# Vanlightly/vsr-tlaplus

Hardware: AMD Instinct MI355X
Metric: distinct states/sec (whole node) + time-to-first-violation, VSR 3-replica (higher is better)
Workload: dtype u64

## Files before the change

vsr_tlaplus_amd/csrc/vsr_kernels.hpp:

```cpp
#pragma once
#include <hip/hip_runtime.h>

#include "vsr_actions.hpp"
#include "vrst_actions.hpp"
#include "vras_actions.hpp"

namespace vsr {

template <int MODEL>
struct ModelOps;
template <>
struct ModelOps<0> {
  template <bool GUARD_ONLY, typename PTR>
  static VSR_HD bool gen_(const Model& M, PTR rec, int ord, Delta& D) { return gen<GUARD_ONLY>(M, rec, ord, D); }
  template <typename PTR>
  static VSR_HD u32 guard_pre(const Model& M, PTR rec, u64 hdr, const u64* Areg, int slot, int* kind0, int info) {
    return guard_slot_pre(M, rec, hdr, Areg, slot, kind0, info);
  }
  template <typename PTR>
  static VSR_HD u32 guard(const Model& M, PTR rec, int slot, int* kind0) { return guard_slot(M, rec, slot, kind0); }
  static VSR_HD int other_kind(int) { return A_SendGetState; }
  template <typename PTR>
  static VSR_HD void hash_child_(const Model& M, PTR rec, const Delta& D, u64* Hc) { hash_child(M, rec, D, Hc); }
  template <typename PTR>
// ... 218 lines not shown
        if (cur == 0) {
          r.slot = lb + k;
          r.claimed = true;
          return r;
        }
        if (cur == fp) {
          r.slot = lb + k;
          r.reload = true;
          return r;
        }
        continue;
      }
      if (cur == fp) {
        r.slot = lb + k;
        r.meta = sk.y;
        return r;
      }
    }
    i = (lb + 4) & mask;
  }
  r.full = true;
  return r;
}

template <typename CNT>
__device__ __forceinline__ bool probe_lookup(const Slot* table, u64 mask, u64 fp, u64* meta, CNT nprobe, u64* slot_out = nullptr) {
  typedef u64 u64x2 __attribute__((ext_vector_type(2)));
  u64 i = fp & mask;
  {
    const u64x2 sk = *(const u64x2*)&table[i];
    nprobe.home();
    if (sk.x == fp) {
      *meta = sk.y;
      if (slot_out) *slot_out = i;
      return true;
    }
    if (sk.x == 0) return false;
    i = (i + 1) & mask;
  }
  for (u32 lines = 0; lines < 2048; lines++) {
    const u64 lb = i & ~(u64)3;
    const u64x2* lp = (const u64x2*)&table[lb];
    const u64x2 s0 = lp[0], s1 = lp[1], s2 = lp[2], s3 = lp[3];
#pragma unroll
    for (int k = 0; k < 4; k++) {
      if (lb + k < i) continue;
      const u64x2 sk = k == 0 ? s0 : k == 1 ? s1 : k == 2 ? s2 : s3;
      nprobe.extra();
      if (sk.x == fp) {
        *meta = sk.y;
        if (slot_out) *slot_out = lb + k;
        return true;
      }
      if (sk.x == 0) return false;
    }
    i = (lb + 4) & mask;
  }
  return false;
}

template <typename CNT>
__device__ __forceinline__ u64 table_claim(Slot* table, u64 mask, u64 fp, u64 key, int level, bool* found_old,
                                           CNT nprobe, bool* full) {
  const Probe p = probe_insert(table, mask, fp, nprobe);
  *full = p.full;
  *found_old = true;
  if (p.full) return 0;
  if (!p.claimed) {
    const u64 m = p.reload ? __hip_atomic_load(&table[p.slot].meta, __ATOMIC_RELAXED, __HIP_MEMORY_SCOPE_AGENT) : p.meta;
    if (meta_level(m) < level || m < key) return p.slot;
  }
  const u64 prev = atomicMin((unsigned long long*)&table[p.slot].meta, (unsigned long long)key);
  *found_old = prev < key;
  return p.slot;
}

template <typename CNT>
__device__ __forceinline__ void table_claim_fused(Slot* table, u64 mask, u64 fp, u64 key, int level, bool* claimed, u64* prev_meta,
                                                  CNT nprobe, bool* full) {
  const Probe p = probe_insert(table, mask, fp, nprobe);
  *full = p.full;
  *claimed = p.claimed;
  *prev_meta = META_EMPTY;
  if (p.full) return;
  if (!p.claimed) {
    const u64 m = p.reload ? __hip_atomic_load(&table[p.slot].meta, __ATOMIC_RELAXED, __HIP_MEMORY_SCOPE_AGENT) : p.meta;
    if (meta_level(m) < level) return;
    if (m != META_EMPTY && m < key) {
      *prev_meta = m;
      return;
    }
  }
  *prev_meta = atomicMin((unsigned long long*)&table[p.slot].meta, (unsigned long long)key);
}

template <int SPEC>
__device__ __forceinline__ void specialise(Model& M, const Model& Marg) {
  constexpr int MODEL = SPEC / 1000, S = SPEC % 1000;
  if constexpr (S != 0) {
    constexpr int SR = S / 100, SC = (S / 10) % 10, SN = S % 10;
    M.R = SR;
    M.C = SC;
    M.n = SN;
    if constexpr (MODEL == 0) {
      M.wpr = 1 + (SR + 2) / 2;
      M.m0 = 4 * SR + SR * SC * SN;
      if (Marg.np == 1) M.np = 1;
      else M.np = SN == 1 ? 1 : SN == 2 ? 2 : 6;
    } else {
      M.wpr = MODEL == 1 ? 1 : 2;
      M.m0 = 4 * SR + SR * SN;
      M.np = 1;
    }
    M.h0 = 1 + SR * M.wpr;
    M.fixed = M.h0 + M.np + VSR_PAD_WORDS;
    M.pitab[0] = 0x24u;
    if (SN == 2) M.pitab[1] = 0x21u;
    if (SN == 3) { M.pitab[1] = 0x18u; M.pitab[2] = 0x21u; M.pitab[3] = 0x09u; M.pitab[4] = 0x12u; M.pitab[5] = 0x06u; }
  }
}

constexpr int EXPAND_GENERAL = 0;
constexpr int EXPAND_PLAIN = 1;
constexpr int EXPAND_MODES = 2;
constexpr int EXPAND_REGEN_BITS = 3;
constexpr int EXPAND_INSERT = 4;
constexpr int EXPAND_PLAIN5 = 5;
constexpr int EXPAND_PROBE = 6;
constexpr int expand_occ(bool fused, int spec, int plain) {
  return !fused ? 3 : spec == 0 ? 2 : (plain == EXPAND_PLAIN5 || plain == EXPAND_PROBE) ? VSR_OCC + 1 : VSR_OCC;
}
template <bool FUSED, int SPEC = 0, int PLAIN = EXPAND_GENERAL>
__global__ void __launch_bounds__(VSR_BLOCK, expand_occ(FUSED, SPEC, PLAIN))
k_expand(Model Marg, const u64* __restrict__ fr_words, const u64* __restrict__ fr_off, u64 n_parents, int level, int rank,
         Slot* table, u64 tmask, u64* pending, u64 pending_cap, LevelCtl* ctl, int stride, int world_arg, u64* cand_send,
         u64 cand_cap, u32 pchunk ,
         u64* nx_words, u64 nx_words_cap, u64* nx_off, u64 nx_cap, u64* lvl_fp, u32 ichunk, u32 wchunk, int tile, u32 ccap ,
         u64* filter, u64 fmask, u64* cand_idx, u32 cchunk ,
         int mode_arg, u64 p_offset ,
         const WSet* wset, u32 wepoch) {
  constexpr bool IS_PLAIN = PLAIN == EXPAND_PLAIN || PLAIN == EXPAND_PLAIN5;
  const int mode = IS_PLAIN ? (int)MODE_NORMAL : PLAIN == EXPAND_REGEN_BITS ? (int)MODE_REGEN : PLAIN == EXPAND_INSERT ? (int)MODE_INSERT
                 : PLAIN == EXPAND_PROBE ? (int)MODE_PROBE : (mode_arg & 0xFF);
  const bool no_footprint = !IS_PLAIN && PLAIN != EXPAND_PROBE && (mode_arg & MODE_NO_FOOTPRINT) != 0;
  const int world = PLAIN != EXPAND_GENERAL ? 1 : world_arg;
  Model M = Marg;
  specialise<SPEC>(M, Marg);
  typedef ModelOps<SPEC / 1000> Ops;
  extern __shared__ u64 smem[];
  u64* s_rec = smem;
  u32* s_cand = (u32*)(smem + tile * stride);
  u32* s_cand2 = s_cand + ccap;
  __shared__ u32 s_ncand, s_napply, s_dead, s_maxbag, s_maxbag_out, s_skip, s_nsurv, s_risky, s_ntotal;
  constexpr int TILE_MAX = (FUSED && SPEC % 1000 != 0 && (SPEC % 1000) / 100 <= 3) ? 64 : VSR_TILE_MAX;
  constexpr bool COOP = FUSED && IS_PLAIN;
  constexpr bool REDO_OK = FUSED && (IS_PLAIN || PLAIN == EXPAND_PROBE);
  __shared__ u32 s_alive[TILE_MAX];
  __shared__ u64 s_ref[TILE_MAX];
  __shared__ u64 s_pfp[TILE_MAX];
  __shared__ u32 s_kcount[16], s_kbase[16];
  __shared__ int s_slotinfo[64];
  __shared__ unsigned long long s_fxs[2];
  __shared__ unsigned long long s_acc[32];
  __shared__ u64 s_chunk_base;
  __shared__ u32 s_chunk_used, s_tile_base, s_tile_cursor;
  __shared__ u64 s_ich_base, s_wch_base;
  __shared__ u32 s_ich_used, s_wch_used, s_tile_ibase, s_tile_wbase, s_tile_icur, s_tile_wcur, s_wneed;
  __shared__ unsigned long long s_cstate[8];
  constexpr bool fused = FUSED;
  constexpr u64 CS_NONE = ((u64)1 << 40) - 1;

  const int tid = threadIdx.x, lane = tid & 63;
#if VSR_WAVE_DIAG
  u64 wd_wait = 0;
  const u64 wd_t0 = __builtin_readcyclecounter();
  __shared__ unsigned long long s_wd[8];
  if (tid < 8) s_wd[tid] = 0;
#endif
  const u64 ntiles = (n_parents + tile - 1) / tile;
  const int tshift = 31 - __clz(tile);
  if (tid < 32) s_acc[tid] = 0;
  if (tid < 2) s_fxs[tid] = 0;
  if (tid == 0) s_maxbag_out = 0;
  if (tid < 64) s_slotinfo[tid] = (SPEC / 1000 == 0 && tid < M.m0) ? slot_info(M, tid) : 0;
  if (tid == 0) {
    s_chunk_base = 0; s_chunk_used = pchunk;
    s_ich_base = 0; s_ich_used = ichunk; s_wch_base = 0; s_wch_used = wchunk;
  }
  if (tid < 8) s_cstate[tid] = (CS_NONE << 24) | cchunk;
  VSR_SYNC_G(0);

  __shared__ u64 s_tile_cur;
  u64 my_next = 0;
  __shared__ u32 s_tile_left;
  const u32 tbatch = ntiles >= (u64)gridDim.x * 16 ? (u32)VSR_TILE_BATCH : 1u;
  if (tid == 0) { my_next = atomicAdd((unsigned long long*)&ctl->tile_cursor, 1ull) * (u64)tbatch; s_tile_left = tbatch - 1; }
  __shared__ u32 s_over;
  if (tid == 0) s_over = 0;
  for (;;) {
    if (tid == 0) {
      s_tile_cur = my_next;
      if (my_next < ntiles) {
        const u32 left = s_tile_left;
        if (left) { my_next++; s_tile_left = left - 1; }
        else { my_next = atomicAdd((unsigned long long*)&ctl->tile_cursor, 1ull) * (u64)tbatch; s_tile_left = tbatch - 1; }
      }
    }
    const u64 t_0 = VSR_CLK();
    if (tid == 0) { s_ncand = 0; s_dead = 0; s_maxbag = 0; s_wneed = 0; s_skip = 0; s_nsurv = 0; s_over = 0; if (!IS_PLAIN) s_risky = 0; }
    if (tid < tile) s_alive[tid] = 0;
    if (tid < 16) s_kcount[tid] = 0;
    VSR_SYNC_G(0);
    u64 tile_i = s_tile_cur;
    tile_i = ((u64)(u32)__builtin_amdgcn_readfirstlane((int)(u32)(tile_i >> 32)) << 32) | (u32)__builtin_amdgcn_readfirstlane((int)(u32)tile_i);
    if (tile_i >= ntiles) break;
    u64 p_base = tile_i * (u64)tile;
    int np_tile = (int)((n_parents - p_base) < (u64)tile ? (n_parents - p_base) : (u64)tile);
    if constexpr (REDO_OK) {
      if (mode_arg & MODE_REDO_LIST) {
        const u64 e = ((const u64*)p_offset)[tile_i >> 1];
        const int cnt = (int)(e >> 48);
        int half = 1;
        while (half * 2 < cnt) half *= 2;
        p_base = (e & (((u64)1 << 48) - 1)) + ((tile_i & 1) ? (u64)half : 0);
        np_tile = (tile_i & 1) ? cnt - half : half;
      }
      p_base = ((u64)(u32)__builtin_amdgcn_readfirstlane((int)(u32)(p_base >> 32)) << 32) | (u32)__builtin_amdgcn_readfirstlane((int)(u32)p_base);
      np_tile = __builtin_amdgcn_readfirstlane(np_tile);
    }
    u32 cbits[2] = {0u, 0u};
    if constexpr (PLAIN == EXPAND_REGEN_BITS) {
      const int pm = tid & (tile - 1), gg = tid >> tshift, GG = VSR_BLOCK >> tshift;
      if (pm < np_tile) {
        const u32* row = (const u32*)filter + (p_offset + p_base + (u64)pm) * fmask;
#pragma unroll
        for (int q = 0; q < 2; q++)
          if ((u64)(gg + q * GG) < fmask) cbits[q] = row[gg + q * GG];
      }
    }

    if (tid < np_tile) {
      const u64 ref = fr_off[p_base + tid];
      s_ref[tid] = ref;
      if (ref) atomicMax(&s_maxbag, (u32)((int)(ref & 255) - M.fixed));
      if ((int)(ref & 255) > stride) raise_error(ctl, ERR_INTERNAL, (p_base + (u64)tid) << 16);
    }
    constexpr int SG = VSR_BLOCK / 16;
    for (int half = 0; half < tile; half += 4 * SG)
      for (int wbase = 0; wbase < stride; wbase += 64) {
        u64 v[4][4];
        u64 refq[4];
#pragma unroll
        for (int q = 0; q < 4; q++) {
          const int p = half + (tid >> 4) + SG * q;
          refq[q] = p < np_tile ? fr_off[p_base + (u64)p] : 0;
        }
#pragma unroll
        for (int q = 0; q < 4; q++) {
          const u64 ref = refq[q];
          const u64 off = ref >> 8;
          const int len = (int)(ref & 255) < stride ? (int)(ref & 255) : stride;
#pragma unroll
          for (int j = 0; j < 4; j++) {
            const int k = wbase + (tid & 15) + 16 * j;
            v[q][j] = k < len ? fr_words[off + k] : 0;
          }
        }
#pragma unroll
        for (int q = 0; q < 4; q++) {
          const int p = half + (tid >> 4) + SG * q;
          const int len = (int)(refq[q] & 255) < stride ? (int)(refq[q] & 255) : stride;
#pragma unroll
          for (int j = 0; j < 4; j++) {
            const int k = wbase + (tid & 15) + 16 * j;
            if (k < len) s_rec[p * stride + k] = v[q][j];
          }
        }
      }
    VSR_SYNC_G(2);
    if (tid < np_tile && s_ref[tid] != 0) {
      const u64* r0 = s_rec + tid * stride;
      u64 pf;
      u32 pa;
      canonical_fp(M, r0[0], r0 + M.h0, &pf, &pa);
      s_pfp[tid] = pf;
    }

    const u64 t_1 = VSR_CLK();
    {
      const int nslots = M.m0 + (int)s_maxbag;
      const int nitems = nslots << tshift;
      const int p_mine = tid & (tile - 1);
      const bool mine_valid = p_mine < np_tile && s_ref[p_mine] != 0;
      const u64* rec_mine = s_rec + p_mine * stride;
      u64 Areg[6] = {0, 0, 0, 0, 0, 0};
      u64 hdr_mine = 0;
      if (mine_valid) {
        hdr_mine = rec_mine[0];
#pragma unroll
        for (int r = 1; r <= 5; r++)
          if (r <= M.R) Areg[r] = rec_mine[1 + (r - 1) * M.wpr];
      }
      const u32 PRIV = PLAIN == EXPAND_PROBE ? 0u : (ccap - (u32)VSR_BLOCK) / VSR_BLOCK;
      const u32 shared0 = PRIV * VSR_BLOCK;
      for (u32 k = tid; k < ccap; k += VSR_BLOCK) s_cand[k] = ~0u;
      VSR_SYNC_G(3);
      u32 nmine = 0;
      bool alive = false;
      if constexpr (SPEC / 1000 == 0) {
        auto emit = [&](int kind, int p, int ord) {
          atomicAdd(&s_kcount[kind], 1u);
          if constexpr (PLAIN == EXPAND_PROBE) {
            if (!((Ops::probe_actions() >> kind) & 1u)) { s_alive[p] = 1; return; }
          }
          u32 idx;
          if (nmine < PRIV) idx = (u32)tid * PRIV + nmine;
          else idx = shared0 + atomicAdd(&s_ncand, 1u);
          nmine++;
          if (idx < ccap) s_cand[idx] = ((u32)kind << 18) | ((u32)p << 11) | (u32)ord;
          else s_ncand = 0x40000000u;
          s_alive[p] = 1;
        };
        const int G = VSR_BLOCK >> tshift, g = tid >> tshift;
        if constexpr (PLAIN == EXPAND_REGEN_BITS) {
          if (mine_valid) {
#pragma unroll
            for (int q = 0; q < 2; q++) {
              u32 bits = cbits[q];
              while (bits) {
                const int b = __ffs((int)bits) - 1;
                bits &= bits - 1;
                const int ord = 32 * (g + q * G) + b;
                int kind;
                if (ord < M.m0) {
                  kind = ord < M.R ? A_TimerSendSVC : ord < 2 * M.R ? A_SendDVC : ord < 3 * M.R ? A_SendSV : ord < 4 * M.R ? A_ExecuteOp : A_ReceiveClientRequest;
                } else {
                  const int q2 = ord - M.m0, j = q2 / (M.R + 1), k2 = q2 - j * (M.R + 1);
                  int kind0 = 0;
                  (void)Ops::guard(M, rec_mine, M.m0 + j, &kind0);
                  kind = k2 == 0 ? kind0 : Ops::other_kind(kind0);
                }
                emit(kind, p_mine, ord);
              }
            }
          }
        } else {
        u64 lut[6] = {0, 0, 0, 0, 0, 0};
        if (mine_valid) {
#pragma unroll
          for (int r = 1; r <= 5; r++)
            if (r <= M.R) lut[r] = prefilter_lut(M, Areg[r], r);
          for (int r = g + 1; r <= M.R; r += G) {
            u32 m = rep_slots_mask(M, rec_mine, hdr_mine, areg_of(Areg, r), r);
            while (m) {
              const int b = __ffs((int)m) - 1;
              m &= m - 1;
              const int kind = b == 0 ? A_TimerSendSVC : b == 1 ? A_SendDVC : b == 2 ? A_SendSV : b == 3 ? A_ExecuteOp : A_ReceiveClientRequest;
              emit(kind, p_mine, b < 4 ? b * M.R + (r - 1) : 4 * M.R + (r - 1) * M.C * M.n + (b - 4));
            }
          }
        }
        u16* s_surv = (u16*)s_cand2;
        const int nmsg_mine = mine_valid ? hdr_nmsg(hdr_mine) : 0;
        const int maxbag = (int)s_maxbag;
        const int jbatch = (int)((2u * ccap) >> tshift);
        for (int j0 = 0; j0 < maxbag; j0 += jbatch) {
          const int j1 = j0 + jbatch < maxbag ? j0 + jbatch : maxbag;
          for (int jj = j0; jj < j1; jj += G) {
            const int j = jj + g;
            bool pass = false;
            if (j < j1 && j < nmsg_mine) {
              const u64 w = rec_mine[M.fixed + j];
              const int r = m_dest(w);
              const u64 l = r == 1 ? lut[1] : r == 2 ? lut[2] : r == 3 ? lut[3] : r == 4 ? lut[4] : lut[5];
              pass = m_count(w) != 0 && ((l >> (w & 63)) & 1);
              if (!IS_PLAIN && PLAIN != EXPAND_REGEN_BITS && PLAIN != EXPAND_INSERT && mode == MODE_PROBE && m_count(w) == 3) s_risky = 1;
            }
            const u64 bal = __ballot(pass);
            if (bal) {
              u32 base = 0;
              if (lane == 0) base = atomicAdd(&s_nsurv, (u32)__popcll(bal));
              base = (u32)__builtin_amdgcn_readfirstlane((int)base);
              if (pass) s_surv[base + (u32)__popcll(bal & (((u64)1 << lane) - 1))] = (u16)((p_mine << 8) | j);
            }
          }
          VSR_SYNC_G(4);
          const u32 nsurv = s_nsurv;
          for (u32 i = tid; i < nsurv; i += VSR_BLOCK) {
            const int p = s_surv[i] >> 8, j = s_surv[i] & 255;
            int kind0 = 0;
            u32 mask = Ops::guard(M, s_rec + p * stride, M.m0 + j, &kind0);
            const int ordbase = M.m0 + j * (M.R + 1);
            while (mask) {
              const int k = __ffs((int)mask) - 1;
              mask &= mask - 1;
              emit(k == 0 ? kind0 : Ops::other_kind(kind0), p, ordbase + k);
            }
          }
          if (j1 < maxbag) {
            VSR_SYNC_G(4);
            if (tid == 0) s_nsurv = 0;
            VSR_SYNC_G(4);
          }
        }
        }
      } else
      {
      for (int item0 = tid; item0 < nitems; item0 += 4 * VSR_BLOCK) {
        u32 masks[4];
        int kinds[4];
#pragma unroll
        for (int u = 0; u < 4; u++) {
          const int item = item0 + u * VSR_BLOCK;
          const int slot = item >> tshift;
          masks[u] = 0;
          kinds[u] = 0;
          if (item < nitems && mine_valid) masks[u] = Ops::guard_pre(M, rec_mine, hdr_mine, Areg, slot, &kinds[u], s_slotinfo[slot & 63]);
        }
#pragma unroll
        for (int u = 0; u < 4; u++) {
          u32 mask = masks[u];
          if (!mask) continue;
          const int slot = (item0 + u * VSR_BLOCK) >> tshift;
          const int ordbase = slot < M.m0 ? slot : M.m0 + (slot - M.m0) * (M.R + 1);
          alive = true;
          while (mask) {
            const int k = __ffs((int)mask) - 1;
            mask &= mask - 1;
            const int kind = k == 0 ? kinds[u] : Ops::other_kind(kinds[u]);
            atomicAdd(&s_kcount[kind], 1u);
            u32 idx;
            if (nmine < PRIV) idx = (u32)tid * PRIV + nmine;
            else idx = shared0 + atomicAdd(&s_ncand, 1u);
            nmine++;
            if (idx < ccap) s_cand[idx] = ((u32)kind << 18) | ((u32)p_mine << 11) | (u32)(ordbase + k);
            else s_ncand = 0x40000000u;
          }
        }
      }
      if (alive) s_alive[p_mine] = 1;
      }
    }
    VSR_SYNC_G(5);
    if (tid < np_tile && s_alive[tid] == 0 && s_ref[tid] != 0) atomicAdd(&s_dead, 1u);
    if (tid == 0) {
      if (s_ncand >= 0x40000000u) {
        bool listed = false;
        if constexpr (REDO_OK) {
          if (np_tile > 1) {
            const u64 k = atomicAdd((unsigned long long*)&ctl->n_redo, 1ull);
            if (k < ctl->redo_cap) { ((u64*)ctl->redo_out)[k] = p_base | ((u64)np_tile << 48); listed = true; s_over = 1; }
          }
        }
        if (!listed) raise_error(ctl, ERR_FRONTIER_FULL, p_base);
      }
      u32 acc = 0;
      if constexpr (!IS_PLAIN && FUSED) {
        const u32 keep = (mode == MODE_PROBE && !no_footprint) ? Ops::probe_actions() : ~0u;
        for (int a = 0; a < 16; a++)
          if ((keep >> a) & 1u) {
            s_kbase[a] = acc;
            acc += s_kcount[a];
          }
        s_napply = acc > ccap ? ccap : acc;
        if (keep != ~0u) {
          for (int a = 0; a < 16; a++)
            if (!((keep >> a) & 1u)) {
              s_kbase[a] = acc;
              acc += s_kcount[a];
            }
          if (!s_over && (s_risky || (int)s_maxbag + M.R - 1 > M.max_bag)) s_acc[15] += acc - s_napply;
        }
      } else {
        for (int a = 0; a < 16; a++) {
          s_kbase[a] = acc;
          acc += s_kcount[a];
        }
      }
      s_ncand = acc > ccap ? ccap : acc;
      if constexpr (PLAIN == EXPAND_PROBE) { s_ntotal = acc; s_ncand = s_napply; }
      if (fused) s_wneed = s_ncand * (u32)(M.fixed + (int)s_maxbag + 5);
    }
    const u64 t_2 = VSR_CLK();
    VSR_SYNC_G(6);
    const u32 ncand = s_ncand;
    if constexpr (REDO_OK) {
      if (s_over) {
        VSR_SYNC_G(6);
        continue;
      }
    }
    for (u32 c = tid; c < ccap; c += VSR_BLOCK) {
      const u32 code = s_cand[c];
      if (code == ~0u) continue;
      const u32 pos = atomicAdd(&s_kbase[code >> 18], 1u);
      if (pos < ccap) s_cand2[pos] = code;
    }
    VSR_SYNC_G(6);

    const u64 t_3 = VSR_CLK();
    if (fused && (mode == MODE_NORMAL || mode == MODE_REGEN)) {
      if (s_ich_used + ncand > ichunk) {
        const u32 used = s_ich_used;
        const u64 base = s_ich_base;
        for (u32 k = used + tid; k < ichunk; k += VSR_BLOCK) {
          nx_off[base + k] = 0;
          lvl_fp[base + k] = 0;
        }
        VSR_SYNC_G(6);
        if (tid == 0) {
          u64 nb = atomicAdd((unsigned long long*)&ctl->n_new, (unsigned long long)ichunk);
          if (nb + ichunk > nx_cap) { raise_full(ctl, nb); nb = 0; }
          s_ich_base = nb;
          s_ich_used = 0;
        }
        VSR_SYNC_G(6);
      }
      if (s_wch_used + s_wneed > wchunk) {
        VSR_SYNC_G(6);
        if (tid == 0) {
          u64 nb = atomicAdd((unsigned long long*)&ctl->words_new, (unsigned long long)wchunk);
          if (nb + wchunk > nx_words_cap) { raise_full(ctl, nb); nb = 0; }
          if (s_wneed > wchunk) { raise_error(ctl, ERR_FRONTIER_FULL, p_base); s_skip = 1; }
          s_wch_base = nb;
          s_wch_used = 0;
        }
        VSR_SYNC_G(6);
      }
      if (tid == 0) { s_tile_ibase = s_ich_used; s_tile_wbase = s_wch_used; s_tile_icur = 0; s_tile_wcur = 0; }
    } else
    if (!fused && s_chunk_used + ncand > pchunk) {
      const u32 used = s_chunk_used;
      const u64 base = s_chunk_base;
      for (u32 k = used + tid; k < pchunk && used < pchunk; k += VSR_BLOCK) pending[3 * (base + k) + 1] = ~(u64)0;
      VSR_SYNC_G(6);
      if (tid == 0) {
        u64 nb = atomicAdd((unsigned long long*)&ctl->n_pending, (unsigned long long)pchunk);
        if (nb + pchunk > pending_cap) {
          raise_error(ctl, ERR_FRONTIER_FULL, nb);
          nb = 0;
        }
        s_chunk_base = nb;
        s_chunk_used = 0;
      }
      VSR_SYNC_G(6);
    }
    const u32 ncand_apply = s_skip ? 0u : ((!IS_PLAIN && FUSED) ? s_napply : ncand);
    if (tid == 0) { s_tile_base = s_chunk_used; s_tile_cursor = 0; }
    VSR_SYNC_G(6);
    const CntLds my_probes{&s_acc[2]};
    for (u32 c = tid; c < ncand_apply; c += VSR_BLOCK) {
      const u32 code = s_cand2[c];
      const int p = (int)((code >> 11) & 127), ord = (int)(code & 2047);
      const u64* rec = s_rec + p * stride;
      Delta D;
      const u64 a_0 = VSR_CLK();
      if (!Ops::template gen_<false>(M, rec, ord, D) || D.action != (int)(code >> 18)) {
        raise_error(ctl, ERR_INTERNAL, ((p_base + (u64)p) << 16) | (u64)ord);
        continue;
      }
      if (D.err) {
        raise_error(ctl, D.err, ((p_base + (u64)p) << 16) | (u64)ord);
        continue;
      }
      if constexpr (PLAIN == EXPAND_PROBE) {
        if (Ops::invariants(M, rec, D) != 0) {
          const u64 i = atomicAdd((unsigned long long*)&ctl->n_pending, 1ull);
          if (i < pending_cap) { pending[2 * i] = origin_make(p_base + (u64)p, ord); pending[2 * i + 1] = 0; }
        }
        continue;
      }
      const u64 a_1 = VSR_CLK();
      if (!IS_PLAIN && fused && mode == MODE_PROBE && Ops::invariants(M, rec, D) == 0) continue;
      u64 Hc[6];
      Ops::hash_child_(M, rec, D, Hc);
      u64 fp;
      u32 ak;
      canonical_fp(M, D.hdr, Hc, &fp, &ak);
      const u64 key = meta_make(level, ak, s_pfp[p]);
      const u64 a_2 = VSR_CLK();
      if (tid == 0) { s_acc[10] += a_1 - a_0; s_acc[11] += a_2 - a_1; }
      if (!fused && world > 1) {
        const int owner = owner_of(fp, world);
        if (owner != rank) {
          for (int o = 0; o < world; o++)
            if (owner == o) {
              u64 i = wave_alloc(&ctl->cand_cnt[o]);
              if (i < cand_cap) {
                cand_send[2 * ((u64)o * cand_cap + i)] = fp;
                cand_send[2 * ((u64)o * cand_cap + i) + 1] = key;
                cand_idx[(u64)o * cand_cap + i] = origin_make(p_offset + p_base + (u64)p, ord);
              } else {
                raise_error(ctl, ERR_FRONTIER_FULL, i);
              }
            }
          continue;
        }
      }
      if (fused) {
        bool do_write = false, remote = false, check = false, claimed_now = false;
        u64 prev_meta = META_EMPTY;
        const int owner = world > 1 ? owner_of(fp, world) : rank;
        if (mode == MODE_PROBE) {
          u64 m = META_EMPTY;
          check = !(probe_lookup(table, tmask, fp, &m, my_probes) && meta_level(m) < level);
          if (!check) continue;
        } else if (owner != rank) {
          if (mode != MODE_REGEN) {
            u64 tag = fp ^ ((u64)(ak + 1) * 0x9E3779B97F4A7C15ull);
            if (tag == 0) tag = 1;
            u64* fs = filter + ((fp >> 6) & fmask);
            if (__hip_atomic_load(fs, __ATOMIC_RELAXED, __HIP_MEMORY_SCOPE_AGENT) == tag) continue;
            __hip_atomic_store(fs, tag, __ATOMIC_RELAXED, __HIP_MEMORY_SCOPE_AGENT);
            remote = true;
            do_write = mode == MODE_NORMAL;
          } else if (wset) {
            do_write = wset_take(wset, fp, level, wepoch);
          } else {
            remote = true;
          }
        } else if (mode == MODE_REGEN && PLAIN == EXPAND_GENERAL && wset) {
          do_write = wset_take(wset, fp, level, wepoch);
        } else if (PLAIN == EXPAND_REGEN_BITS) {
          do_write = (((const u32*)filter)[(p_offset + p_base + (u64)p) * fmask + ((u32)ord >> 5)] >> ((u32)ord & 31u)) & 1u;
        } else if (mode == MODE_REGEN) {
          u64 m = META_EMPTY;
          u64 slot_i = 0;
          do_write = probe_lookup(table, tmask, fp, &m, my_probes, &slot_i) && m == key &&
                     atomicCAS((unsigned long long*)&table[slot_i].meta, (unsigned long long)key, (unsigned long long)(key | META_TAKEN)) == key;
        } else {
          bool claimed, full;
          table_claim_fused(table, tmask, fp, key, level, &claimed, &prev_meta, my_probes, &full);
          if (full) {
            raise_error(ctl, ERR_TABLE_FULL, fp);
            continue;
          }
          do_write = claimed;
          claimed_now = claimed;
          if (PLAIN == EXPAND_GENERAL && wset && claimed && !wset_insert(wset, fp, level)) raise_error(ctl, ERR_TABLE_FULL, fp);
          if (PLAIN == EXPAND_INSERT && filter && claimed)
            atomicOr(&((u32*)filter)[(p_offset + p_base + (u64)p) * fmask + ((u32)ord >> 5)], 1u << ((u32)ord & 31u));
        }
        int bad = (check || do_write || (remote && mode == MODE_INSERT)) ? Ops::invariants(M, rec, D) : 0;
#ifdef VSRMC_TEST_HOOKS
        if constexpr (PLAIN == EXPAND_GENERAL)
          if (M.test_bad_mask && fp == M.test_bad_fp && (check || do_write || remote)) bad |= (int)M.test_bad_mask;
#endif
        if (mode == MODE_PROBE) {
          if (bad) {
// ... 16 lines not shown
            }
            atomicMin((unsigned long long*)&ctl->viol_fp, (unsigned long long)fp);
            atomicOr(&ctl->viol_mask, (u32)bad);
          }
          if ((u32)hdr_nmsg(D.hdr) > s_maxbag_out) atomicMax(&s_maxbag_out, (u32)hdr_nmsg(D.hdr));
          atomicAdd(&s_acc[9], 1ull);
          atomicXor(&s_fxs[0], (unsigned long long)fp);
          atomicAdd(&s_fxs[1], (unsigned long long)fp);
          do_write = false;
        }
        const u64 a_3 = VSR_CLK();
        if (tid == 0) s_acc[12] += a_3 - a_2;
        u64 idx = 0;
        u64 dst = 0;
        int plen = 0, clen = 0;
        if (do_write) {
          plen = (int)(s_ref[p] & 255);
          clen = M.fixed + hdr_nmsg(D.hdr);
          const u32 io = atomicAdd(&s_tile_icur, 1u);
          const u32 wo = atomicAdd(&s_tile_wcur, (u32)clen);
          idx = s_ich_base + s_tile_ibase + io;
          dst = s_wch_base + s_tile_wbase + wo;
        }
        if constexpr (COOP) {
          const u64 act = __ballot(1);
          u64 wm = __ballot(do_write);
          const int nact = __popcll(act), rnk = __popcll(act & (((u64)1 << lane) - 1));
          while (wm) {
            const int l0 = __ffsll((long long)wm) - 1;
            wm &= wm - 1;
            const int l1 = wm ? __ffsll((long long)wm) - 1 : l0;
            wm &= wm - 1;
            const int n0 = __builtin_amdgcn_readlane(plen, l0), n1 = l1 != l0 ? __builtin_amdgcn_readlane(plen, l1) : 0;
            const u64* r0 = s_rec + __builtin_amdgcn_readlane(p, l0) * stride;
            const u64* r1 = s_rec + __builtin_amdgcn_readlane(p, l1) * stride;
            u64* o0 = nx_words + readlane64(dst, l0);
            u64* o1 = nx_words + readlane64(dst, l1);
            for (int k = rnk; k < n0 || k < n1; k += nact) {
              const u64 v0 = k < n0 ? r0[k] : 0, v1 = k < n1 ? r1[k] : 0;
              if (k < n0) o0[k] = v0;
              if (k < n1) o1[k] = v1;
            }
          }
        }
        if (do_write) {
          u64* out = nx_words + dst;
          if constexpr (!COOP) {
            typedef u64 u64x2_a8 __attribute__((ext_vector_type(2), aligned(8)));
            int k = 0;
            if (plen - k >= 2) {
              u64x2_a8 cur;
              cur.x = rec[k];
              cur.y = rec[k + 1];
              for (; k + 3 < plen; k += 2) {
                u64x2_a8 nxt;
                nxt.x = rec[k + 2];
                nxt.y = rec[k + 3];
                *(u64x2_a8*)(out + k) = cur;
                cur = nxt;
              }
              *(u64x2_a8*)(out + k) = cur;
              k += 2;
            }
            for (; k + 1 < plen; k += 2) {
              u64x2_a8 v2;
              v2.x = rec[k];
              v2.y = rec[k + 1];
              *(u64x2_a8*)(out + k) = v2;
            }
            if (k < plen) out[k] = rec[k];
          }
          out[0] = D.hdr;
          u64* ob = out + 1 + (D.r - 1) * M.wpr;
          ob[0] = D.rep[0];
          if (M.wpr > 1) ob[1] = D.rep[1];
          if (M.wpr > 2) ob[2] = D.rep[2];
          if (M.wpr > 3) ob[3] = D.rep[3];
#pragma unroll
          for (int k = 0; k < 6; k++)
            if (k < M.np) out[M.h0 + k] = Hc[k];
          int a = 0;
#pragma unroll
          for (int k = 0; k < VSR_NSLOT; k++)
            if ((D.used >> k) & 1) {
              if (D.pj(k) >= 0) out[M.fixed + D.pj(k)] = D.pnew[k];
              else out[plen + (a++)] = D.pnew[k];
            }
          nx_off[idx] = (dst << 8) | (u64)clen;
          lvl_fp[idx] = fp;
          if (bad && !remote) {
            atomicMin((unsigned long long*)&ctl->viol_fp, (unsigned long long)fp);
            atomicOr(&ctl->viol_mask, (u32)bad);
          }
          if ((u32)hdr_nmsg(D.hdr) > s_maxbag_out) atomicMax(&s_maxbag_out, (u32)hdr_nmsg(D.hdr));
        }
        if (PLAIN == EXPAND_GENERAL && remote) {
          u64 i = 0;
          for (;;) {
            const unsigned long long old = atomicAdd(&s_cstate[owner], 1ull);
            const u32 pos = (u32)(old & 0xFFFFFFull);
            if (pos == cchunk) {
              u64 nb = atomicAdd((unsigned long long*)&ctl->cand_cnt[owner], (unsigned long long)cchunk);
              if (nb + cchunk > cand_cap) { raise_error(ctl, ERR_FRONTIER_FULL, nb); nb = 0; }
              const u64 ob_ = (u64)(old >> 24);
              (void)ob_;
              i = nb;
              atomicExch(&s_cstate[owner], ((unsigned long long)nb << 24) | 1ull);
              break;
            }
            if (pos < cchunk) {
              i = (u64)(old >> 24) + pos;
              break;
            }
          }
          const u64 e = (u64)owner * cand_cap + i;
          cand_send[2 * e] = fp;
          cand_send[2 * e + 1] = key;
          cand_idx[e] = mode == MODE_REGEN ? origin_make(p_base + (u64)p, ord)
                                           : cand_pack(mode == MODE_INSERT ? (u64)hdr_nmsg(D.hdr) : idx, (u32)bad);
        }
        if (prev_meta != META_EMPTY && meta_level(prev_meta) == level && meta_auxkey(prev_meta) != meta_auxkey(key)) atomicAdd(&s_acc[8], 1ull);
        if (tid == 0) s_acc[13] += VSR_CLK() - a_3;
        continue;
      }
      bool found_old, full;
      u64 slot = table_claim(table, tmask, fp, key, level, &found_old, my_probes, &full);
      if (full) {
        raise_error(ctl, ERR_TABLE_FULL, fp);
        continue;
      }
      if (!found_old) {
        const u64 active = __ballot(1);
        const int leader = __ffsll((long long)active) - 1;
        u32 b = 0;
        if (lane == leader) b = atomicAdd(&s_tile_cursor, (u32)__popcll(active));
        b = __shfl(b, leader);
        const u64 i = s_chunk_base + s_tile_base + b + (u32)__popcll(active & (((u64)1 << lane) - 1));
        pending[3 * i] = slot;
        pending[3 * i + 1] = key;
        pending[3 * i + 2] = origin_make(p_offset + p_base + (u64)p, ord);
      }
    }
    const u64 t_4 = VSR_CLK();
    VSR_SYNC_G(7);
    if (tid == 0) {
      if (fused) {
        s_ich_used += s_tile_icur;
        s_wch_used += s_tile_wcur;
        s_acc[14] += s_tile_icur;
        if (mode == MODE_NORMAL || mode == MODE_REGEN) s_acc[9] += s_tile_wcur;
      } else {
        s_chunk_used += s_tile_cursor;
      }
      s_acc[0] += PLAIN == EXPAND_PROBE ? s_ntotal : s_ncand;
      s_acc[1] += s_dead;
      if (PLAIN != EXPAND_PROBE) s_acc[2] += ncand_apply;
      const u64 t_5 = VSR_CLK();
      s_acc[3] += t_1 - t_0;
      s_acc[4] += t_2 - t_1;
      s_acc[5] += t_3 - t_2;
      s_acc[6] += t_4 - t_3;
      s_acc[7] += t_5 - t_4;
    }
    if (tid < 16) s_acc[16 + tid] += s_kcount[tid];
  }
  {
    if (fused) {
      const u32 used = s_ich_used;
      const u64 base = s_ich_base;
      for (u32 k = used + tid; k < ichunk; k += VSR_BLOCK) {
        nx_off[base + k] = 0;
        lvl_fp[base + k] = 0;
      }
      if (world > 1) {
        VSR_SYNC_G(0);
        for (int o = 0; o < world; o++) {
          const u64 st = s_cstate[o];
          const u64 base = st >> 24;
          const u32 used = (u32)(st & 0xFFFFFFull) < cchunk ? (u32)(st & 0xFFFFFFull) : cchunk;
          if (base == CS_NONE) continue;
          for (u32 k = used + tid; k < cchunk; k += VSR_BLOCK) {
            cand_send[2 * ((u64)o * cand_cap + base + k)] = 0;
            cand_send[2 * ((u64)o * cand_cap + base + k) + 1] = ~(u64)0;
          }
        }
      }
      if (tid == 0) {
        if (s_acc[8]) atomicAdd((unsigned long long*)&ctl->ties, s_acc[8]);
        if (!IS_PLAIN && s_acc[15]) atomicAdd((unsigned long long*)&ctl->limit_unchecked, s_acc[15]);
        if (s_acc[14]) atomicAdd((unsigned long long*)&ctl->n_written, s_acc[14]);
        if (s_acc[9]) atomicAdd((unsigned long long*)(mode == MODE_INSERT ? &ctl->n_new : &ctl->rec_words), s_acc[9]);
        if (s_maxbag_out) atomicMax((unsigned long long*)&ctl->max_bag, (unsigned long long)s_maxbag_out);
        if (!IS_PLAIN && (s_fxs[0] | s_fxs[1])) {
          atomicXor((unsigned long long*)&ctl->fp_xor, s_fxs[0]);
          atomicAdd((unsigned long long*)&ctl->fp_sum, s_fxs[1]);
        }
      }
    } else {
      const u32 used = s_chunk_used;
      const u64 base = s_chunk_base;
      for (u32 k = used + tid; k < pchunk; k += VSR_BLOCK) pending[3 * (base + k) + 1] = ~(u64)0;
    }
    if (tid == 0) {
      if (s_acc[0]) atomicAdd((unsigned long long*)&ctl->generated, s_acc[0]);
      if (s_acc[1]) atomicAdd((unsigned long long*)&ctl->deadlocks, s_acc[1]);
      if (s_acc[2]) atomicAdd((unsigned long long*)&ctl->probes, s_acc[2]);
    }
#if VSR_WAVE_DIAG == 3
    if (tid == 64) {
      for (int g = 0; g < 8; g++) atomicAdd((unsigned long long*)&ctl->phase_cycles[g], s_wd[g]);
      atomicAdd((unsigned long long*)&ctl->act_generated[0], (unsigned long long)(__builtin_readcyclecounter() - wd_t0));
    }
    (void)wd_wait;
#elif VSR_WAVE_DIAG
    if (lane == 0 && (tid >> 6) < 4) {
      atomicAdd((unsigned long long*)&ctl->phase_cycles[tid >> 6], (unsigned long long)wd_wait);
      atomicAdd((unsigned long long*)&ctl->phase_cycles[4 + (tid >> 6)], (unsigned long long)(__builtin_readcyclecounter() - wd_t0));
    }
#else
    if (tid >= 3 && tid < 8 && s_acc[tid]) atomicAdd((unsigned long long*)&ctl->phase_cycles[tid - 3], s_acc[tid]);
    if (tid >= 10 && tid < 13 && s_acc[tid]) atomicAdd((unsigned long long*)&ctl->phase_cycles[tid - 5], s_acc[tid]);
    if (tid == 13 && s_acc[13]) atomicAdd((unsigned long long*)&ctl->act_generated[0], s_acc[13]);
#endif
    if (tid >= 16 && tid < 32 && s_acc[tid]) atomicAdd((unsigned long long*)&ctl->act_generated[tid - 16], s_acc[tid]);
  }
}

__device__ __forceinline__ void write_child_serial(const Model& M, const u64* rec, const Delta& D, const u64* Hc, u64* dst) {
  int nmsg = hdr_nmsg(rec[0]);
  int len = M.fixed + nmsg;
  for (int k = 0; k < len; k++) dst[k] = rec[k];
  dst[0] = D.hdr;
  for (int k = 0; k < M.wpr; k++) dst[1 + (D.r - 1) * M.wpr + k] = D.rep[k];
  for (int i = 0; i < M.np; i++) dst[M.h0 + i] = Hc[i];
  int a = 0;
#pragma unroll
  for (int k = 0; k < VSR_NSLOT; k++)
    if ((D.used >> k) & 1) {
      if (D.pj(k) >= 0) dst[M.fixed + D.pj(k)] = D.pnew[k];
      else dst[M.fixed + nmsg + (a++)] = D.pnew[k];
    }
}

#define VSR_MAT_BLOCK 64
#define VSR_MAT_GROUP 16

__device__ __forceinline__ void lds_wave_sync() {
  __builtin_amdgcn_fence(__ATOMIC_RELEASE, "workgroup");
  __builtin_amdgcn_wave_barrier();
  __builtin_amdgcn_fence(__ATOMIC_ACQUIRE, "workgroup");
}

template <int SPEC>
__global__ void __launch_bounds__(VSR_MAT_BLOCK)
k_materialize(Model Marg, const u64* __restrict__ fr_words, const u64* __restrict__ fr_off, const u64* __restrict__ pending,
              u64 n_pending, Slot* table, u64* nx_words, u64 nx_words_cap, u64* nx_off, u64 nx_cap,
              u64* lvl_fp, LevelCtl* ctl, const uint8_t* __restrict__ verdict, u64* cnt_n, u64* cnt_w, int stride,
              u32 ichunk , u32 wchunk ,
              int es, const u64* __restrict__ pidx_arr) {
  Model M = Marg;
  specialise<SPEC>(M, Marg);
  typedef ModelOps<SPEC / 1000> Ops;
  extern __shared__ u64 s_slot[];
  const int lane = threadIdx.x;
  u64 idx_base = 0, w_base = 0;
  u32 idx_left = 0, w_left = 0;
  u64 cyc_fetch = 0, cyc_stage = 0, cyc_gen = 0, cyc_write = 0, rec_words = 0;
  const u64 nthreads = (u64)gridDim.x * VSR_MAT_BLOCK;
  const u64 rounds = (n_pending + nthreads - 1) / nthreads;
  for (u64 it = 0; it < rounds; it++) {
    const u64 i = it * nthreads + (u64)blockIdx.x * VSR_MAT_BLOCK + lane;
    const u64 c_0 = __builtin_readcyclecounter();
    bool win = false;
    u64 key = 0, src = 0, origin = 0;
    int plen = 0;
    if (i < n_pending) {
      key = pending[(u64)es * i + 1];
      if (key != ~(u64)0) {
        origin = pidx_arr ? pidx_arr[i] : pending[(u64)es * i + 2];
        const u64 ref = fr_off[origin_pidx(origin)];
        if (verdict) win = verdict[i] != 0;
        else win = atomicCAS((unsigned long long*)&table[pending[(u64)es * i]].meta, (unsigned long long)key,
                             (unsigned long long)(key | META_TAKEN)) == key;
        src = ref >> 8;
        plen = (int)(ref & 255);
        if (plen > stride) plen = stride;
      }
    }
    if (!win) plen = 0;
    const u64 wmask = __ballot(win);
    const u64 c_1 = __builtin_readcyclecounter();
    cyc_fetch += c_1 - c_0;
    if (wmask == 0) continue;
    for (int w = 0; w < 64; w++) {
      const int n2 = 2 * __builtin_amdgcn_readlane(plen, w);
      if (n2 == 0) continue;
      const u32* g = (const u32*)(fr_words + readlane64(src, w));
      __attribute__((address_space(3))) void* l = (__attribute__((address_space(3))) void*)(s_slot + w * stride);
      if (lane < n2) __builtin_amdgcn_global_load_lds((const __attribute__((address_space(1))) void*)(g + lane), l, 4, 0, 0);
      if (lane + 64 < n2) __builtin_amdgcn_global_load_lds((const __attribute__((address_space(1))) void*)(g + lane), l, 4, 256, 0);
      if (lane + 128 < n2) __builtin_amdgcn_global_load_lds((const __attribute__((address_space(1))) void*)(g + lane), l, 4, 512, 0);
      if (lane + 192 < n2) __builtin_amdgcn_global_load_lds((const __attribute__((address_space(1))) void*)(g + lane), l, 4, 768, 0);
    }
    asm volatile("s_waitcnt vmcnt(0)" ::: "memory");
    lds_wave_sync();
    const u64 c_2 = __builtin_readcyclecounter();
    cyc_stage += c_2 - c_1;
// ... 786 lines not shown
```

Measured before the change: 1.777 billion.

## Store private candidate slots column-major and skip full-buffer candidate clearing

```diff
diff --git a/vsr_tlaplus_amd/csrc/vsr_kernels.hpp b/vsr_tlaplus_amd/csrc/vsr_kernels.hpp
--- a/vsr_tlaplus_amd/csrc/vsr_kernels.hpp
+++ b/vsr_tlaplus_amd/csrc/vsr_kernels.hpp
@@ -394,8 +394,12 @@
   u32* s_cand = (u32*)(smem + tile * stride);
   u32* s_cand2 = s_cand + ccap;
   __shared__ u32 s_ncand, s_napply, s_dead, s_maxbag, s_maxbag_out, s_skip, s_nsurv, s_risky, s_ntotal;
+  u32& s_nlist = s_nsurv;
   constexpr int TILE_MAX = (FUSED && SPEC % 1000 != 0 && (SPEC % 1000) / 100 <= 3) ? 64 : VSR_TILE_MAX;
   constexpr bool COOP = FUSED && IS_PLAIN;
+  constexpr bool COLS = SPEC / 1000 == 0;
+  constexpr bool TWO_COLS = FUSED && SPEC != 0 && SPEC / 1000 == 0 && expand_occ(FUSED, SPEC, PLAIN) == VSR_OCC;
+  constexpr bool FLAT_STAGE = PLAIN == EXPAND_REGEN_BITS;
   constexpr bool REDO_OK = FUSED && (IS_PLAIN || PLAIN == EXPAND_PROBE);
   __shared__ u32 s_alive[TILE_MAX];
   __shared__ u64 s_ref[TILE_MAX];
@@ -497,25 +501,51 @@
           const int p = half + (tid >> 4) + SG * q;
           refq[q] = p < np_tile ? fr_off[p_base + (u64)p] : 0;
         }
-#pragma unroll
-        for (int q = 0; q < 4; q++) {
-          const u64 ref = refq[q];
-          const u64 off = ref >> 8;
-          const int len = (int)(ref & 255) < stride ? (int)(ref & 255) : stride;
+        if constexpr (FLAT_STAGE) {
+#pragma unroll
+          for (int q = 0; q < 4; q++) {
+            const u64 ref = refq[q];
+            const u64* src = fr_words + (ref >> 8);
+            const int len = (int)(ref & 255) < stride ? (int)(ref & 255) : stride;
+#pragma unroll
+            for (int j = 0; j < 4; j++) {
+              const int k = wbase + (tid & 15) + 16 * j;
+              v[q][j] = src[k < len ? k : 0];
+            }
+          }
 #pragma unroll
           for (int j = 0; j < 4; j++) {
             const int k = wbase + (tid & 15) + 16 * j;
-            v[q][j] = k < len ? fr_words[off + k] : 0;
+            if (k < stride) {
+#pragma unroll
+              for (int q = 0; q < 4; q++) {
+                const int p = half + (tid >> 4) + SG * q;
+                const int len = (int)(refq[q] & 255);
+                s_rec[p * stride + k] = k < len ? v[q][j] : 0;
+              }
+            }
           }
-        }
-#pragma unroll
-        for (int q = 0; q < 4; q++) {
-          const int p = half + (tid >> 4) + SG * q;
-          const int len = (int)(refq[q] & 255) < stride ? (int)(refq[q] & 255) : stride;
-#pragma unroll
-          for (int j = 0; j < 4; j++) {
-            const int k = wbase + (tid & 15) + 16 * j;
-            if (k < len) s_rec[p * stride + k] = v[q][j];
+        } else {
+#pragma unroll
+          for (int q = 0; q < 4; q++) {
+            const u64 ref = refq[q];
+            const u64 off = ref >> 8;
+            const int len = (int)(ref & 255) < stride ? (int)(ref & 255) : stride;
+#pragma unroll
+            for (int j = 0; j < 4; j++) {
+              const int k = wbase + (tid & 15) + 16 * j;
+              v[q][j] = k < len ? fr_words[off + k] : 0;
+            }
+          }
+#pragma unroll
+          for (int q = 0; q < 4; q++) {
+            const int p = half + (tid >> 4) + SG * q;
+            const int len = (int)(refq[q] & 255) < stride ? (int)(refq[q] & 255) : stride;
+#pragma unroll
+            for (int j = 0; j < 4; j++) {
+              const int k = wbase + (tid & 15) + 16 * j;
+              if (k < len) s_rec[p * stride + k] = v[q][j];
+            }
           }
         }
       }
@@ -529,6 +559,13 @@
     }
 
     const u64 t_1 = VSR_CLK();
+    const u32 PRIV = PLAIN == EXPAND_PROBE ? 0u : (ccap - (u32)VSR_BLOCK) / VSR_BLOCK;
+    const u32 shared0 = PRIV * VSR_BLOCK;
+    if constexpr (!COLS) {
+      for (u32 k = tid; k < ccap; k += VSR_BLOCK) s_cand[k] = ~0u;
+      VSR_SYNC_G(3);
+    }
+    u32 nmine = 0;
     {
       const int nslots = M.m0 + (int)s_maxbag;
       const int nitems = nslots << tshift;
@@ -543,11 +580,6 @@
         for (int r = 1; r <= 5; r++)
           if (r <= M.R) Areg[r] = rec_mine[1 + (r - 1) * M.wpr];
       }
-      const u32 PRIV = PLAIN == EXPAND_PROBE ? 0u : (ccap - (u32)VSR_BLOCK) / VSR_BLOCK;
-      const u32 shared0 = PRIV * VSR_BLOCK;
-      for (u32 k = tid; k < ccap; k += VSR_BLOCK) s_cand[k] = ~0u;
-      VSR_SYNC_G(3);
-      u32 nmine = 0;
       bool alive = false;
       if constexpr (SPEC / 1000 == 0) {
         auto emit = [&](int kind, int p, int ord) {
@@ -556,7 +588,7 @@
             if (!((Ops::probe_actions() >> kind) & 1u)) { s_alive[p] = 1; return; }
           }
           u32 idx;
-          if (nmine < PRIV) idx = (u32)tid * PRIV + nmine;
+          if (nmine < PRIV) idx = nmine * (u32)VSR_BLOCK + (u32)tid;
           else idx = shared0 + atomicAdd(&s_ncand, 1u);
           nmine++;
           if (idx < ccap) s_cand[idx] = ((u32)kind << 18) | ((u32)p << 11) | (u32)ord;
@@ -608,22 +640,50 @@
         const int jbatch = (int)((2u * ccap) >> tshift);
         for (int j0 = 0; j0 < maxbag; j0 += jbatch) {
           const int j1 = j0 + jbatch < maxbag ? j0 + jbatch : maxbag;
-          for (int jj = j0; jj < j1; jj += G) {
-            const int j = jj + g;
-            bool pass = false;
-            if (j < j1 && j < nmsg_mine) {
-              const u64 w = rec_mine[M.fixed + j];
-              const int r = m_dest(w);
-              const u64 l = r == 1 ? lut[1] : r == 2 ? lut[2] : r == 3 ? lut[3] : r == 4 ? lut[4] : lut[5];
-              pass = m_count(w) != 0 && ((l >> (w & 63)) & 1);
-              if (!IS_PLAIN && PLAIN != EXPAND_REGEN_BITS && PLAIN != EXPAND_INSERT && mode == MODE_PROBE && m_count(w) == 3) s_risky = 1;
+          if constexpr (TWO_COLS) {
+            for (int jj = j0; jj < j1; jj += 2 * G) {
+              bool pass[2];
+#pragma unroll
+              for (int u = 0; u < 2; u++) {
+                const int j = jj + u * G + g;
+                pass[u] = false;
+                if (j < j1 && j < nmsg_mine) {
+                  const u64 w = rec_mine[M.fixed + j];
+                  const int r = m_dest(w);
+                  const u64 l = r == 1 ? lut[1] : r == 2 ? lut[2] : r == 3 ? lut[3] : r == 4 ? lut[4] : lut[5];
+                  pass[u] = m_count(w) != 0 && ((l >> (w & 63)) & 1);
+                  if (!IS_PLAIN && PLAIN != EXPAND_REGEN_BITS && PLAIN != EXPAND_INSERT && mode == MODE_PROBE && m_count(w) == 3) s_risky = 1;
+                }
+              }
+              const u64 bal0 = __ballot(pass[0]), bal1 = __ballot(pass[1]);
+              if (bal0 | bal1) {
+                const u32 n0 = (u32)__popcll(bal0);
+                u32 base = 0;
+                if (lane == 0) base = atomicAdd(&s_nsurv, n0 + (u32)__popcll(bal1));
+                base = (u32)__builtin_amdgcn_readfirstlane((int)base);
+                const u64 below = ((u64)1 << lane) - 1;
+                if (pass[0]) s_surv[base + (u32)__popcll(bal0 & below)] = (u16)((p_mine << 8) | (jj + g));
+                if (pass[1]) s_surv[base + n0 + (u32)__popcll(bal1 & below)] = (u16)((p_mine << 8) | (jj + G + g));
+              }
             }
-            const u64 bal = __ballot(pass);
-            if (bal) {
-              u32 base = 0;
-              if (lane == 0) base = atomicAdd(&s_nsurv, (u32)__popcll(bal));
-              base = (u32)__builtin_amdgcn_readfirstlane((int)base);
-              if (pass) s_surv[base + (u32)__popcll(bal & (((u64)1 << lane) - 1))] = (u16)((p_mine << 8) | j);
+          } else {
+            for (int jj = j0; jj < j1; jj += G) {
+              const int j = jj + g;
+              bool pass = false;
+              if (j < j1 && j < nmsg_mine) {
+                const u64 w = rec_mine[M.fixed + j];
+                const int r = m_dest(w);
+                const u64 l = r == 1 ? lut[1] : r == 2 ? lut[2] : r == 3 ? lut[3] : r == 4 ? lut[4] : lut[5];
+                pass = m_count(w) != 0 && ((l >> (w & 63)) & 1);
+                if (!IS_PLAIN && PLAIN != EXPAND_REGEN_BITS && PLAIN != EXPAND_INSERT && mode == MODE_PROBE && m_count(w) == 3) s_risky = 1;
+              }
+              const u64 bal = __ballot(pass);
+              if (bal) {
+                u32 base = 0;
+                if (lane == 0) base = atomicAdd(&s_nsurv, (u32)__popcll(bal));
+                base = (u32)__builtin_amdgcn_readfirstlane((int)base);
+                if (pass) s_surv[base + (u32)__popcll(bal & (((u64)1 << lane) - 1))] = (u16)((p_mine << 8) | j);
+              }
             }
           }
           VSR_SYNC_G(4);
@@ -683,19 +743,21 @@
       if (alive) s_alive[p_mine] = 1;
       }
     }
+    if constexpr (COLS)
+      if (nmine < PRIV) s_cand[nmine * (u32)VSR_BLOCK + (u32)tid] = ~0u;
     VSR_SYNC_G(5);
     if (tid < np_tile && s_alive[tid] == 0 && s_ref[tid] != 0) atomicAdd(&s_dead, 1u);
+    if (tid == 0 && s_ncand >= 0x40000000u) {
+      bool listed = false;
+      if constexpr (REDO_OK) {
+        if (np_tile > 1) {
+          const u64 k = atomicAdd((unsigned long long*)&ctl->n_redo, 1ull);
+          if (k < ctl->redo_cap) { ((u64*)ctl->redo_out)[k] = p_base | ((u64)np_tile << 48); listed = true; s_over = 1; }
+        }
+      }
+      if (!listed) raise_error(ctl, ERR_FRONTIER_FULL, p_base);
+    }
     if (tid == 0) {
-      if (s_ncand >= 0x40000000u) {
-        bool listed = false;
-        if constexpr (REDO_OK) {
-          if (np_tile > 1) {
-            const u64 k = atomicAdd((unsigned long long*)&ctl->n_redo, 1ull);
-            if (k < ctl->redo_cap) { ((u64*)ctl->redo_out)[k] = p_base | ((u64)np_tile << 48); listed = true; s_over = 1; }
-          }
-        }
-        if (!listed) raise_error(ctl, ERR_FRONTIER_FULL, p_base);
-      }
       u32 acc = 0;
       if constexpr (!IS_PLAIN && FUSED) {
         const u32 keep = (mode == MODE_PROBE && !no_footprint) ? Ops::probe_actions() : ~0u;
@@ -719,24 +781,39 @@
           acc += s_kcount[a];
         }
       }
-      s_ncand = acc > ccap ? ccap : acc;
-      if constexpr (PLAIN == EXPAND_PROBE) { s_ntotal = acc; s_ncand = s_napply; }
-      if (fused) s_wneed = s_ncand * (u32)(M.fixed + (int)s_maxbag + 5);
+      s_nlist = acc > ccap ? ccap : acc;
+      if constexpr (PLAIN == EXPAND_PROBE) { s_ntotal = acc; s_nlist = s_napply; }
+      if (fused) s_wneed = s_nlist * (u32)(M.fixed + (int)s_maxbag + 5);
     }
     const u64 t_2 = VSR_CLK();
     VSR_SYNC_G(6);
-    const u32 ncand = s_ncand;
+    const u32 ncand = s_nlist;
     if constexpr (REDO_OK) {
       if (s_over) {
         VSR_SYNC_G(6);
         continue;
       }
     }
-    for (u32 c = tid; c < ccap; c += VSR_BLOCK) {
-      const u32 code = s_cand[c];
-      if (code == ~0u) continue;
-      const u32 pos = atomicAdd(&s_kbase[code >> 18], 1u);
-      if (pos < ccap) s_cand2[pos] = code;
+    if constexpr (!COLS) {
+      for (u32 c = tid; c < ccap; c += VSR_BLOCK) {
+        const u32 code = s_cand[c];
+        if (code == ~0u) continue;
+        const u32 pos = atomicAdd(&s_kbase[code >> 18], 1u);
+        if (pos < ccap) s_cand2[pos] = code;
+      }
+    } else {
+      for (u32 c = tid; c < shared0; c += VSR_BLOCK) {
+        const u32 code = s_cand[c];
+        if (code == ~0u) break;
+        const u32 pos = atomicAdd(&s_kbase[code >> 18], 1u);
+        if (pos < ccap) s_cand2[pos] = code;
+      }
+      const u32 nshared = s_ncand < ccap - shared0 ? s_ncand : ccap - shared0;
+      for (u32 c = tid; c < nshared; c += VSR_BLOCK) {
+        const u32 code = s_cand[shared0 + c];
+        const u32 pos = atomicAdd(&s_kbase[code >> 18], 1u);
+        if (pos < ccap) s_cand2[pos] = code;
+      }
     }
     VSR_SYNC_G(6);
 
@@ -1059,7 +1136,7 @@
       } else {
         s_chunk_used += s_tile_cursor;
       }
-      s_acc[0] += PLAIN == EXPAND_PROBE ? s_ntotal : s_ncand;
+      s_acc[0] += PLAIN == EXPAND_PROBE ? s_ntotal : s_nlist;
       s_acc[1] += s_dead;
       if (PLAIN != EXPAND_PROBE) s_acc[2] += ncand_apply;
       const u64 t_5 = VSR_CLK();
```

Result: no change. 1.791 billion (median of 6 runs) (+0.8%).
